# AllenNeuralDynamics/aind-smartspim-destripe

Measured on AMD Instinct MI355X. Metric: 2048x2048 uint16 slices/s destriped, higher is better.
Workload: dtype f32

## Files before the change

### aind_smartspim_destripe_amd/csrc/dsx_kernels.h

```cpp
#ifndef DSX_KERNELS_H
#define DSX_KERNELS_H

#include <type_traits>
#include <hip/hip_runtime.h>
#include <stdint.h>

#include "dsx_fft_core.h"

#ifndef DSX_NT
#define DSX_NT 1
#endif
#ifndef DSX_MEDIAN_BALLOT
#define DSX_MEDIAN_BALLOT 1
#endif
#ifndef DSX_FWD_STEADY
#define DSX_FWD_STEADY 1
#endif
#ifndef DSX_RF_XCD
#define DSX_RF_XCD 0
#endif
#ifndef DSX_INV_MINW
#define DSX_INV_MINW 1
#endif
#ifndef DSX_FWD_PRUNE
#define DSX_FWD_PRUNE 1
#endif
#ifndef DSX_SWZ
#define DSX_SWZ 1
#endif
#ifndef DSX_FWD_MINW
#define DSX_FWD_MINW 4
#endif


#ifdef DSX_DIAG
#define DSX_ABL(a, bits) (((a).ablate & (bits)) != 0)
#else
#define DSX_ABL(a, bits) false
#endif

namespace dsx {

constexpr int kMaxLevels = 16;
constexpr int kMaxPasses = 16;
constexpr int kWave = 64;

#define DSX_DEC_LO                                                                              \
  {0.03522629188570953f, -0.08544127388202666f, -0.13501102001025458f, 0.45987750211849154f,   \
   0.8068915093110925f,  0.33267055295008263f}
#define DSX_DEC_HI                                                                              \
  {-0.33267055295008263f, 0.8068915093110925f,  -0.45987750211849154f, -0.13501102001025458f,  \
   0.08544127388202666f,  0.03522629188570953f}
#define DSX_REC_LO                                                                              \
  {0.33267055295008263f,  0.8068915093110925f,   0.45987750211849154f, -0.13501102001025458f,  \
   -0.08544127388202666f, 0.03522629188570953f}
#define DSX_REC_HI                                                                              \
  {0.03522629188570953f, 0.08544127388202666f, -0.13501102001025458f, -0.45987750211849154f,   \
   0.8068915093110925f,  -0.33267055295008263f}

typedef unsigned dsx_u32x2 __attribute__((ext_vector_type(2)));
typedef float dsx_f2 __attribute__((ext_vector_type(2)));
typedef float dsx_f4 __attribute__((ext_vector_type(4)));
typedef unsigned dsx_u32x4 __attribute__((ext_vector_type(4)));

__device__ __forceinline__ __amdgpu_buffer_rsrc_t dsx_rsrc(const void* p) {
  return __builtin_amdgcn_make_buffer_rsrc((void*)p, 0, -1, 0x00020000);
}
constexpr int kBufNT = 2;

#if DSX_SCALAR_FMA
__device__ __forceinline__ dsx_f2 pk_fma(dsx_f2 a, dsx_f2 b, dsx_f2 c) { return dsx_f2{fmaf(a.x, b.x, c.x), fmaf(a.y, b.y, c.y)}; }
__device__ __forceinline__ dsx_f2 pk_fma(dsx_f2 a, float b, dsx_f2 c) { return dsx_f2{fmaf(a.x, b, c.x), fmaf(a.y, b, c.y)}; }
__device__ __forceinline__ dsx_f2 pk_fma(float a, dsx_f2 b, dsx_f2 c) { return dsx_f2{fmaf(a, b.x, c.x), fmaf(a, b.y, c.y)}; }
#else
__device__ __forceinline__ dsx_f2 pk_fma(dsx_f2 a, dsx_f2 b, dsx_f2 c) { return __builtin_elementwise_fma(a, b, c); }
__device__ __forceinline__ dsx_f2 pk_fma(dsx_f2 a, float b, dsx_f2 c) {
  const dsx_f2 bb = {b, b};
  return __builtin_elementwise_fma(a, bb, c);
}
__device__ __forceinline__ dsx_f2 pk_fma(float a, dsx_f2 b, dsx_f2 c) {
  const dsx_f2 aa = {a, a};
  return __builtin_elementwise_fma(aa, b, c);
}
#endif

struct PlaneStats {
  double sum_fg;
  double sum_all;
  unsigned long long cnt_fg;
  unsigned long long flags;
  unsigned pad_[56];
};
static_assert(sizeof(PlaneStats) == 256, "control block layout");

__device__ __forceinline__ int reflect_idx(int i, int n) {
  if (i >= 0 && i < n) return i;
  int p = 2 * n;
  i %= p;
  if (i < 0) i += p;
  return i < n ? i : p - 1 - i;
}

__device__ __forceinline__ float as_f32(unsigned u) { return __uint_as_float(u); }
__device__ __forceinline__ unsigned as_u32(float f) { return __float_as_uint(f); }

__device__ __forceinline__ double wave_sum_f64(double v) {
#pragma unroll
  for (int o = 32; o > 0; o >>= 1) v += __shfl_xor(v, o);
  return v;
}
__device__ __forceinline__ float wave_max_f32(float v) {
#pragma unroll
  for (int o = 32; o > 0; o >>= 1) v = fmaxf(v, __shfl_xor(v, o));
  return v;
}
__device__ __forceinline__ float wave_min_f32(float v) {
#pragma unroll
  for (int o = 32; o > 0; o >>= 1) v = fminf(v, __shfl_xor(v, o));
  return v;
}

__device__ __forceinline__ float min_no_nan(float a, float b) {
  float r;
  asm("v_min_f32 %0, %1, %2" : "=v"(r) : "v"(a), "v"(b));
  return r;
}
__device__ __forceinline__ float max_no_nan(float a, float b) {
  float r;
  asm("v_max_f32 %0, %1, %2" : "=v"(r) : "v"(a), "v"(b));
  return r;
}
__device__ __forceinline__ float wave_min_no_nan(float v) {
  v = min_no_nan(v, __builtin_bit_cast(float, __builtin_amdgcn_update_dpp(0, __builtin_bit_cast(int, v), 0xB1, 0xF, 0xF, true)));
  v = min_no_nan(v, __builtin_bit_cast(float, __builtin_amdgcn_update_dpp(0, __builtin_bit_cast(int, v), 0x4E, 0xF, 0xF, true)));
  v = min_no_nan(v, __builtin_bit_cast(float, __builtin_amdgcn_update_dpp(0, __builtin_bit_cast(int, v), 0x141, 0xF, 0xF, true)));
  v = min_no_nan(v, __builtin_bit_cast(float, __builtin_amdgcn_update_dpp(0, __builtin_bit_cast(int, v), 0x140, 0xF, 0xF, true)));
  const int b = __builtin_bit_cast(int, v);
  const float r0 = __builtin_bit_cast(float, __builtin_amdgcn_readlane(b, 0)), r1 = __builtin_bit_cast(float, __builtin_amdgcn_readlane(b, 16));
  const float r2 = __builtin_bit_cast(float, __builtin_amdgcn_readlane(b, 32)), r3 = __builtin_bit_cast(float, __builtin_amdgcn_readlane(b, 48));
  return fminf(fminf(r0, r1), fminf(r2, r3));
}

__device__ __forceinline__ unsigned swap_adjacent(unsigned v) {
  return (unsigned)__builtin_amdgcn_mov_dpp((int)v, 0xB1, 0xF, 0xF, true);
}

template <typename M>
__device__ __forceinline__ int slot_mask(M m, int e) {
  const unsigned w = (sizeof(M) == 8 && e >= 32) ? (unsigned)((unsigned long long)m >> 32) : (unsigned)m;
  return (int)(w << (31 - (e & 31))) >> 31;
}
template <typename M>
__device__ __forceinline__ M opaque_mask(M m) {
  if constexpr (sizeof(M) == 8) {
    unsigned lo = (unsigned)m, hi = (unsigned)((unsigned long long)m >> 32);
    asm volatile("" : "+v"(lo), "+v"(hi));
    return (M)(((unsigned long long)hi << 32) | lo);
  } else {
    unsigned lo = (unsigned)m;
    asm volatile("" : "+v"(lo));
    return (M)lo;
  }
}
__device__ __forceinline__ unsigned bit_select(int m, unsigned a, unsigned b) {
  unsigned r;
  asm("v_bfi_b32 %0, %1, %2, %3" : "=v"(r) : "v"(m), "v"(a), "v"(b));
  return r;
}
__device__ __forceinline__ int odd_lane_mask(int lane) {
  int m = -(lane & 1);
  asm("" : "+v"(m));
  return m;
}
__device__ __forceinline__ float bit_select(int m, float a, float b) {
  return as_f32(bit_select(m, as_u32(a), as_u32(b)));
}

__device__ __forceinline__ void wave_sync() {
  __builtin_amdgcn_fence(__ATOMIC_RELEASE, "wavefront");
  __builtin_amdgcn_wave_barrier();
  __builtin_amdgcn_fence(__ATOMIC_ACQUIRE, "wavefront");
}

#ifndef DSX_SCALAR_FMA
#define DSX_SCALAR_FMA 1
#endif
#ifndef DSX_FWD_PAIR
#define DSX_FWD_PAIR 1
#endif
#ifndef DSX_FWD_SPLIT
#define DSX_FWD_SPLIT 1
#endif
#ifndef DSX_DPP_X
#define DSX_DPP_X 1
#endif
__device__ __forceinline__ float lane_above(float v) {
  return __builtin_bit_cast(float, __builtin_amdgcn_update_dpp(0, __builtin_bit_cast(int, v), 0x130, 0xF, 0xF, true));
}

__global__ __launch_bounds__(256) void k_zero3(uint4* p0, int n0, uint4* p1, int n1, uint4* p2, int n2) {
  const uint4 z = make_uint4(0u, 0u, 0u, 0u);
  for (int i = blockIdx.x * 256 + threadIdx.x; i < n0 + n1 + n2; i += gridDim.x * 256) {
    if (i < n0) p0[i] = z;
    else if (i < n0 + n1) p1[i - n0] = z;
    else p2[i - n0 - n1] = z;
  }
}

struct Fwd1Args {
  const void* in;
  long long in_plane_stride;
  float* ws;
  long long ws_plane_stride;
  long long in_off;
  int H, W, ldin;
  long long aa_off, da_off;
  int h, w, ld, lda;
  unsigned* minmax;
  int lvl, L;
  PlaneStats* stats;
  float fg_cutoff;
  unsigned fg_cutoff_u16;
  int nstrips, nseg, rows_per_seg;
  long long aa2_off, da2_off;
  int h2, w2, ld2, lda2;
  int ablate;
  int shared;
};

constexpr int kMarchCols = 256;
constexpr int kMarchOut = (kMarchCols - 4) / 2;
constexpr int kFuseOut = (kMarchOut - 4) / 2;
constexpr int kRingRows = 8;
constexpr int kRingPitch = 128;
constexpr int kX2Pitch = 136;

template <int IN_KIND>
struct MarchStats {
  unsigned cnt = 0;
  unsigned isum_all = 0, isum_fg = 0;
  double fsum_all = 0.0, fsum_fg = 0.0;
  unsigned bad = 0;
  __device__ __forceinline__ void add(float f, float cutoff) {
    if (IN_KIND != 0) bad |= (f > -1.0f && f <= 3.402823466e38f) ? 0u : 1u;
    if (IN_KIND == 0) {
      const unsigned u = (unsigned)f;
      isum_all += u;
      if (f >= cutoff) { isum_fg += u; cnt++; }
    } else {
      fsum_all += (double)f;
      if (f >= cutoff) { fsum_fg += (double)f; cnt++; }
    }
  }
};

struct MarchRaw {
  float4 f;
};

struct MarchCol {
  int gc0;
  int base;
  bool vec;
  bool rev;
  bool dead;
  bool own;
  unsigned own_mask[2];
  int rc[4];
};

__device__ __forceinline__ MarchCol march_col(int gc0, int W, int ld, int w_out, bool lane_owns, bool ext) {
  MarchCol c;
  c.gc0 = gc0;
  c.own = lane_owns;
  c.dead = gc0 > 2 * w_out - 1;
  c.rev = false;
  c.base = gc0;
  const bool aligned = (ld & 3) == 0;
  c.vec = aligned && gc0 >= 0 && gc0 + 3 < W;
  if (ext && aligned && gc0 >= -4 && gc0 + 3 < W + 8) c.vec = true;
  if (!c.vec && !ext && aligned && (W & 3) == 0) {
    if (gc0 + 3 < 0 && -gc0 - 1 < W) { c.base = -gc0 - 4; c.rev = true; c.vec = true; }
    else if (gc0 >= W && 2 * W - 4 - gc0 >= 0) { c.base = 2 * W - 4 - gc0; c.rev = true; c.vec = true; }
  }
  if (c.dead) { c.base = 0; c.rev = false; }
  c.own_mask[0] = c.own_mask[1] = 0u;
#pragma unroll
  for (int e = 0; e < 4; ++e) {
    c.rc[e] = reflect_idx(gc0 + e, W);
    if (lane_owns && gc0 + e >= 0 && gc0 + e < W) c.own_mask[e >> 1] |= (e & 1) ? 0xFFFF0000u : 0x0000FFFFu;
  }
  return c;
}

template <int IN_KIND>
struct MarchSrc {
  static constexpr int ES = (IN_KIND == 0) ? 2 : 4;
  static constexpr int BIAS = (IN_KIND == 2) ? 4 : 0;
  const void* src;
  __amdgpu_buffer_rsrc_t rs;
  unsigned voff;
  __device__ __forceinline__ MarchSrc(const void* p, const MarchCol& c)
      : src(p), rs(dsx_rsrc((const char*)p - BIAS * ES)), voff((unsigned)(c.base + BIAS) * ES) {}
  __device__ __forceinline__ MarchRaw load(unsigned soff) const {
    MarchRaw r;
    if (IN_KIND == 0) {
      const dsx_u32x2 u = __builtin_amdgcn_raw_buffer_load_b64(rs, voff, soff, 0);
      r.f = make_float4(__uint_as_float(u.x), __uint_as_float(u.y), 0.f, 0.f);
    } else {
      const dsx_u32x4 u = __builtin_amdgcn_raw_buffer_load_b128(rs, voff, soff, 0);
      r.f = make_float4(__uint_as_float(u.x), __uint_as_float(u.y), __uint_as_float(u.z), __uint_as_float(u.w));
    }
    return r;
  }
};

// ... 903 lines not shown
template <int CPL, int M_, int S_, int R, int... REST>
__device__ __forceinline__ void fft_static_passes_swz(float2* buf, const float2* tw, int lane_in) {
  int lane = lane_in;
  asm volatile("" : "+v"(lane));
#if DSX_SWZ == 2
  fft_pass<R, CPL, (R - 1) / 2, (R - 1) / 2, dsx_idx_swz>(buf, tw, M_, S_, 1.0f / (float)S_, lane);
#else
  fft_pass_swz<R, CPL, M_, S_>(buf, tw, lane);
#endif
  if constexpr (sizeof...(REST) > 0) fft_static_passes_swz<CPL, M_, S_ * R, REST...>(buf, tw, lane_in);
}
template <int PLAN_>
struct StaticFft {
  static constexpr int M = 0;
  static constexpr bool kSwz = false;
};
template <>
struct StaticFft<1> {
  static constexpr int M = 1026;
  static constexpr bool kSwz = false;
  static constexpr int kRadix[3] = {19, 9, 6};
  template <int CPL>
  static __device__ __forceinline__ void run(float2* buf, const float2* tw, int lane) {
    fft_static_passes<CPL, 1026, 1, 19, 9, 6>(buf, tw, lane);
  }
#if DSX_FWD_PRUNE
  template <int CPL, int KO>
  static __device__ __forceinline__ void run_last_pruned(float2* buf, const float2* tw, int lane_in) {
    fft_static_passes<CPL, 1026, 1, 6, 9>(buf, tw, lane_in);
    int lane = lane_in;
    asm volatile("" : "+v"(lane));
    fft_pass<19, CPL, 9, KO>(buf, tw, 1026, 54, 1.0f / 54.0f, lane);
  }
  template <int CPL>
  static __device__ __forceinline__ void run_forward(float2* buf, const float2* tw, int lane, int kcut) {
    const int ko = (kcut + 53) / 54;
    if (ko <= 2) run_last_pruned<CPL, 2>(buf, tw, lane);
    else if (ko <= 4) run_last_pruned<CPL, 4>(buf, tw, lane);
    else run<CPL>(buf, tw, lane);
  }
#else
  template <int CPL>
  static __device__ __forceinline__ void run_forward(float2* buf, const float2* tw, int lane, int) { run<CPL>(buf, tw, lane); }
#endif
  template <int CPL, int JK>
  static __device__ __forceinline__ void run_first_pruned(float2* buf, const float2* tw, int lane_in) {
    int lane = lane_in;
    asm volatile("" : "+v"(lane));
    fft_pass<19, CPL, JK>(buf, tw, 1026, 1, 1.0f, lane);
    fft_static_passes<CPL, 1026, 19, 9, 6>(buf, tw, lane_in);
  }
  template <int CPL>
  static __device__ __forceinline__ void run_inverse(float2* buf, const float2* tw, int lane, int kcut) {
    const int jk = (kcut + 53) / 54;
    if (jk <= 2) run_first_pruned<CPL, 2>(buf, tw, lane);
    else if (jk <= 4) run_first_pruned<CPL, 4>(buf, tw, lane);
    else run<CPL>(buf, tw, lane);
  }
};
template <>
struct StaticFft<2> {
  static constexpr int M = 1071;
  static constexpr bool kSwz = false;
  static constexpr int kRadix[3] = {17, 9, 7};
  template <int CPL>
  static __device__ __forceinline__ void run(float2* buf, const float2* tw, int lane) {
    fft_static_passes<CPL, 1071, 1, 17, 9, 7>(buf, tw, lane);
  }
  template <int CPL>
  static __device__ __forceinline__ void run_forward(float2* buf, const float2* tw, int lane, int) { run<CPL>(buf, tw, lane); }
  template <int CPL>
  static __device__ __forceinline__ void run_inverse(float2* buf, const float2* tw, int lane, int) {
    run<CPL>(buf, tw, lane);
  }
};

#define DSX_STATIC_FFT(ID, LEN, R0, R1, R2, SWZ)                                                   \
  template <>                                                                                      \
  struct StaticFft<ID> {                                                                           \
    static constexpr int M = LEN;                                                                  \
    static constexpr bool kSwz = SWZ;                                                              \
    template <int CPL>                                                                             \
    static __device__ __forceinline__ void run(float2* buf, const float2* tw, int lane) {          \
      if constexpr (SWZ) fft_static_passes_swz<CPL, LEN, 1, R0, R1, R2>(buf, tw, lane);            \
      else fft_static_passes<CPL, LEN, 1, R0, R1, R2>(buf, tw, lane);                              \
    }                                                                                              \
    template <int CPL>                                                                             \
    static __device__ __forceinline__ void run_forward(float2* buf, const float2* tw, int lane, int) { \
      run<CPL>(buf, tw, lane);                                                                     \
    }                                                                                              \
    template <int CPL>                                                                             \
    static __device__ __forceinline__ void run_inverse(float2* buf, const float2* tw, int lane, int) { \
      run<CPL>(buf, tw, lane);                                                                     \
    }                                                                                              \
  };
DSX_STATIC_FFT(3, 2048, 16, 16, 8, DSX_SWZ != 0)
DSX_STATIC_FFT(4, 1815, 15, 11, 11, false)
DSX_STATIC_FFT(5, 1024, 16, 8, 8, DSX_SWZ != 0)
DSX_STATIC_FFT(6, 960, 15, 8, 8, false)
#undef DSX_STATIC_FFT

typedef short dsx_s16x2 __attribute__((ext_vector_type(2)));

__device__ __forceinline__ dsx_s16x2 as_s16x2(unsigned u) {
  union { unsigned u; dsx_s16x2 v; } c;
  c.u = u;
  return c.v;
}
__device__ __forceinline__ unsigned as_u32(dsx_s16x2 v) {
  union { unsigned u; dsx_s16x2 v; } c;
  c.v = v;
  return c.u;
}

template <int CPL>
struct RowSlots {
  static constexpr int GV = CPL / 4;
  static constexpr int E = 4 * GV + 4;
};
template <int E>
struct SlotMask { typedef unsigned long long type; };
template <> struct SlotMask<4> { typedef unsigned type; };
template <> struct SlotMask<8> { typedef unsigned type; };
template <> struct SlotMask<12> { typedef unsigned type; };
template <> struct SlotMask<20> { typedef unsigned type; };

template <int GV, typename F>
__device__ __forceinline__ void for_slots(int gf, int nt, F&& f) {
#pragma unroll
  for (int g = 0; g < GV; ++g) {
    if (g < gf) {
#pragma unroll
      for (int i = 0; i < 4; ++i) f(4 * g + i);
    }
  }
#pragma unroll
  for (int k = 0; k < 4; ++k) {
    if (k < nt) f(4 * GV + k);
  }
}

template <int GV, int E>
__device__ __forceinline__ unsigned count_below_pk16(const unsigned (&x)[E], unsigned t, int gf, int nt) {
  const dsx_s16x2 tv = as_s16x2(t);
  dsx_s16x2 acc = as_s16x2(0u);
  for_slots<GV>(gf, nt, [&](int e) {
    const dsx_s16x2 d = __builtin_elementwise_sub_sat(as_s16x2(x[e]), tv);
    acc -= (d >> 15);
  });
  return as_u32(acc);
}

template <int GV, int E>
__device__ __forceinline__ unsigned bisect_pk16(const unsigned (&x)[E], unsigned rank_a, unsigned rank_b,
                                                int gf, int nt) {
  unsigned ra = 0, rb = 0;
  for (int bit = 15; bit >= 0; --bit) {
    const unsigned ta = ra | (1u << bit), tb = rb | (1u << bit);
    unsigned c = count_below_pk16<GV, E>(x, (ta | (tb << 16)) ^ 0x80008000u, gf, nt);
    c = __reduce_add_sync(~0ull, c);
    if ((c & 0xFFFFu) <= rank_a) ra = ta;
    if ((c >> 16) <= rank_b) rb = tb;
  }
  return ra | (rb << 16);
}

template <int CPL>
constexpr int row_waves_per_simd() {
  return CPL <= 18 ? 4 : 1;
}
constexpr int kRowMaxWaves = 8;

__host__ __device__ __forceinline__ constexpr int rf_lds_row_b(int M) { return (M + 1) & ~1; }

template <int CPL, int GF_, int NT_, int HALO_, int PLAN_, bool TO_LDS>
__device__ __forceinline__ void rf_pair_body(const RowArgs& a, float2* s_tw, float2* buf, int tid, int nthreads, int lane,
                                             int pair, int plane) {
  const int M = (PLAN_ > 0) ? StaticFft<PLAN_>::M : a.M;
  constexpr bool SWZ = StaticFft<PLAN_>::kSwz;
  auto P = [](int i) { return SWZ ? dsx_idx_swz::at(i) : i; };
  const int N = a.w, K = (HALO_ == 0) ? 0 : a.K;
  const bool halo = (HALO_ >= 0) ? (HALO_ != 0) : (K > 0);
  const int npairs = (a.h + 1) >> 1;
  const bool live = pair < npairs;
  const int r0 = live ? 2 * pair : 0;
  const bool has_b = (r0 + 1) < a.h;
  const int cfg = a.cfg[plane];
  float* rowa = a.ws + plane * a.ws_plane_stride + a.da_off + (long long)r0 * a.ld;
  float* rowb = rowa + a.ld;

  constexpr int GV = RowSlots<CPL>::GV;
  constexpr int E = RowSlots<CPL>::E;
  typedef typename SlotMask<E>::type mask_t;
  const int gf = (GF_ >= 0) ? GF_ : (N >> 8);
  const int tail0 = gf << 8;
  const int nt = (NT_ >= 0) ? NT_ : ((N - tail0 + 63) >> 6);
  const int tn = tail0 + lane;

  const bool inactive = a.lvl >= a.lvl_active[cfg];
  auto zero_rows = [&]() {
    if (live) {
      for (int n = 4 * lane; n < N; n += 4 * kWave) {
        *(float4*)(rowa + n) = make_float4(0.f, 0.f, 0.f, 0.f);
        if (has_b) *(float4*)(rowb + n) = make_float4(0.f, 0.f, 0.f, 0.f);
      }
    }
  };
  if (!TO_LDS && inactive) {
    zero_rows();
    return;
  }
  const bool active = live && !inactive;
  const float thr = a.thr[(long long)plane * a.L + a.lvl];

  float4 ra4[GV > 0 ? GV : 1], rb4[GV > 0 ? GV : 1];
  float rta[4], rtb[4];
#pragma unroll
  for (int g = 0; g < GV; ++g) {
    ra4[g] = make_float4(0.f, 0.f, 0.f, 0.f);
    rb4[g] = make_float4(0.f, 0.f, 0.f, 0.f);
    if (active && g < gf) {
      ra4[g] = *(const float4*)(rowa + 256 * g + 4 * lane);
      if (has_b) rb4[g] = *(const float4*)(rowb + 256 * g + 4 * lane);
    }
  }
#pragma unroll
  for (int k = 0; k < 4; ++k) {
    rta[k] = 0.f;
    rtb[k] = 0.f;
    if (active && k < nt && tn + 64 * k < N) {
      rta[k] = rowa[tn + 64 * k];
      if (has_b) rtb[k] = rowb[tn + 64 * k];
    }
  }
  for (int i = tid; i < M; i += nthreads) s_tw[P(i)] = a.tw[i];
  __syncthreads();
  float* const lds_a = (float*)buf;
  float* const lds_b = (float*)buf + rf_lds_row_b(M);
  if (!active) {
    if (TO_LDS) {
      for (int n = 2 * lane; n < N; n += 2 * kWave) {
        *(float2*)(lds_a + n) = make_float2(0.f, 0.f);
        *(float2*)(lds_b + n) = make_float2(0.f, 0.f);
      }
    }
    return;
  }

  float va[E], vb[E];
  mask_t maska = 0, maskb = 0;
  auto take = [&](int e, float xa, float xb, bool valid) {
    const bool ma = valid && fabsf(xa) > thr, mb = valid && fabsf(xb) > thr;
    if (ma) maska |= ((mask_t)1 << e);
    if (mb) maskb |= ((mask_t)1 << e);
    va[e] = valid ? (ma ? 0.f : xa) : __builtin_huge_valf();
    vb[e] = valid ? (mb ? 0.f : xb) : __builtin_huge_valf();
  };
#pragma unroll
  for (int g = 0; g < GV; ++g) {
    if (g < gf) {
      take(4 * g + 0, ra4[g].x, rb4[g].x, true);
      take(4 * g + 1, ra4[g].y, rb4[g].y, true);
      take(4 * g + 2, ra4[g].z, rb4[g].z, true);
      take(4 * g + 3, ra4[g].w, rb4[g].w, true);
    }
  }
#pragma unroll
  for (int k = 0; k < 4; ++k) {
    if (k < nt) take(4 * GV + k, rta[k], rtb[k], tn + 64 * k < N);
  }
  if (!has_b) {
    for_slots<GV>(gf, nt, [&](int e) { if (vb[e] != __builtin_huge_valf()) vb[e] = 0.f; });
  }

  float meda = 0.f, medb = 0.f;
  const bool any_mask = __ballot((maska | maskb) != (mask_t)0) != 0ull;
  if (any_mask && !DSX_ABL(a, 1)) {
    const unsigned k1 = (unsigned)(N - 1) >> 1;
    const bool even = (N & 1) == 0;
    auto count2 = [&](float ta, float tb, bool le) -> unsigned {
#if DSX_MEDIAN_BALLOT
      unsigned ca = 0, cb = 0;
      for_slots<GV>(gf, nt, [&](int e) {
        ca += (unsigned)__popcll(__ballot(le ? (va[e] <= ta) : (va[e] < ta)));
        cb += (unsigned)__popcll(__ballot(le ? (vb[e] <= tb) : (vb[e] < tb)));
      });
      return ca | (cb << 16);
#else
      unsigned ca = 0, cb = 0;
      for_slots<GV>(gf, nt, [&](int e) {
        ca += (le ? (va[e] <= ta) : (va[e] < ta)) ? 1u : 0u;
        cb += (le ? (vb[e] <= tb) : (vb[e] < tb)) ? 1u : 0u;
      });
      return (unsigned)__builtin_amdgcn_readfirstlane((int)__reduce_add_sync(~0ull, ca | (cb << 16)));
#endif
    };
    float lo[2], hi[2];
    unsigned clo[2], chi[2];
    bool done[2];
    float flo[2], fhi[2];
    int last[2] = {0, 0};
    const float target = (float)k1 + 0.5f;
    const float thr_up = as_f32(as_u32(thr) + 1u);
    {
      const unsigned c0 = count2(0.f, 0.f, false), c0e = count2(0.f, 0.f, true);
#pragma unroll
      for (int r = 0; r < 2; ++r) {
        const unsigned lt = r ? (c0 >> 16) : (c0 & 0xFFFFu), le = r ? (c0e >> 16) : (c0e & 0xFFFFu);
        done[r] = false;
        if (k1 < lt) {
          lo[r] = -thr; clo[r] = 0u; hi[r] = 0.f; chi[r] = lt;
        } else if (k1 < le) {
          lo[r] = 0.f; clo[r] = lt; hi[r] = as_f32(1u); chi[r] = le; done[r] = true;
        } else {
          lo[r] = as_f32(1u); clo[r] = le; hi[r] = thr_up; chi[r] = (unsigned)N;
        }
        flo[r] = (float)clo[r] - target;
        fhi[r] = (float)chi[r] - target;
      }
    }
    bool adj[2] = {done[0], done[1]};
    for (int it = 0; it < 256; ++it) {
      const bool fin0 = adj[0] || chi[0] - clo[0] <= 1u, fin1 = adj[1] || chi[1] - clo[1] <= 1u;
      if (fin0 && fin1) break;
      float t[2];
#pragma unroll
      for (int r = 0; r < 2; ++r) {
        float tt = (lo[r] * fhi[r] - hi[r] * flo[r]) * __builtin_amdgcn_rcpf(fhi[r] - flo[r]);
        if ((it & 7) == 7 || !(tt > lo[r] && tt < hi[r])) {
          const unsigned kl = f32_key(lo[r]), kh = f32_key(hi[r]);
          if (kh - kl <= 1u) adj[r] = true;
          tt = key_f32(kl + ((kh - kl) >> 1));
        }
        t[r] = tt;
      }
      const unsigned c = count2(t[0], t[1], false);
#pragma unroll
      for (int r = 0; r < 2; ++r) {
        const unsigned cr = r ? (c >> 16) : (c & 0xFFFFu);
        const float f = (float)cr - target;
        if (cr <= k1) {
          lo[r] = t[r]; clo[r] = cr; flo[r] = f;
          if (last[r] == 1) fhi[r] *= 0.5f;
          last[r] = 1;
        } else {
          hi[r] = t[r]; chi[r] = cr; fhi[r] = f;
          if (last[r] == 2) flo[r] *= 0.5f;
          last[r] = 2;
        }
      }
    }
    float m_lo[2] = {__builtin_huge_valf(), __builtin_huge_valf()}, m_hi[2] = {__builtin_huge_valf(), __builtin_huge_valf()};
    for_slots<GV>(gf, nt, [&](int e) {
      m_lo[0] = min_no_nan(m_lo[0], va[e] >= lo[0] ? va[e] : __builtin_huge_valf());
      m_lo[1] = min_no_nan(m_lo[1], vb[e] >= lo[1] ? vb[e] : __builtin_huge_valf());
      if (even) {
        m_hi[0] = min_no_nan(m_hi[0], va[e] >= hi[0] ? va[e] : __builtin_huge_valf());
        m_hi[1] = min_no_nan(m_hi[1], vb[e] >= hi[1] ? vb[e] : __builtin_huge_valf());
      }
    });
    float sk[2], sk1[2];
#pragma unroll
    for (int r = 0; r < 2; ++r) {
      sk[r] = wave_min_no_nan(m_lo[r]);
      sk1[r] = sk[r];
      if (even) {
        const float nxt = wave_min_no_nan(m_hi[r]);
        sk1[r] = (k1 + 1u < chi[r]) ? sk[r] : nxt;
      }
    }
    meda = even ? 0.5f * (sk[0] + sk1[0]) : sk[0];
    medb = even ? 0.5f * (sk[1] + sk1[1]) : sk[1];
  }
  asm volatile("" : "+v"(meda), "+v"(medb));

  for_slots<GV>(gf, nt, [&](int e) {
    const int n = (e < 4 * GV) ? 256 * (e >> 2) + 4 * lane + (e & 3) : tn + 64 * (e - 4 * GV);
    if (e < 4 * GV || n < N) {
      const float xa = bit_select(slot_mask(maska, e), meda, va[e]);
      const float xb = bit_select(slot_mask(maskb, e), medb, vb[e]);
      const float2 z = make_float2(xa, xb);
      buf[P(K + n)] = z;
      if (halo) {
        if (n <= K) buf[P(K + N + n)] = z;
        if (n >= N - K) buf[P(n - (N - K))] = z;
      }
    }
  });
  if (halo) {
    for (int m = N + 2 * K + 1 + lane; m < M; m += kWave) buf[P(m)] = make_float2(0.f, 0.f);
  }
  wave_sync();

  if (!DSX_ABL(a, 2)) {
    if constexpr (PLAN_ > 0) StaticFft<PLAN_>::template run_forward<CPL>(buf, s_tw, lane, a.kcut[cfg]);
    else fft_run<CPL>(buf, s_tw, a, lane);
  }

  if (!DSX_ABL(a, 4)) {
    const float2* g1 = a.g[cfg];
    const float2* g2 = g1 + M;
    const int kcut = a.kcut[cfg];
    for (int k = lane; k <= kcut; k += kWave) {
      const int kr = (k == 0) ? 0 : M - k;
      const float2 u = buf[P(k)], ur = buf[P(kr)];
      const float ga = g1[k].x;
      const float2 gb = g2[k];
      const float2 v = make_float2(ga * u.x + gb.x * ur.x - gb.y * ur.y, ga * u.y + gb.x * ur.y + gb.y * ur.x);
      const float2 vr = make_float2(ga * ur.x + gb.x * u.x + gb.y * u.y, ga * ur.y + gb.x * u.y - gb.y * u.x);
      buf[P(k)] = make_float2(v.y, v.x);
      if (kr != k) buf[P(kr)] = make_float2(vr.y, vr.x);
    }
    for (int k = kcut + 1 + lane; k < M - kcut; k += kWave) buf[P(k)] = make_float2(0.f, 0.f);
    wave_sync();
  }

  if (!DSX_ABL(a, 2)) {
    if constexpr (PLAN_ > 0) StaticFft<PLAN_>::template run_inverse<CPL>(buf, s_tw, lane, a.kcut[cfg]);
    else fft_run<CPL>(buf, s_tw, a, lane);
  }

  maska = opaque_mask(maska);
  maskb = opaque_mask(maskb);
  if (TO_LDS) {
    float oa[E], ob[E];
    const int no_b = has_b ? 0 : -1;
    for_slots<GV>(gf, nt, [&](int e) {
      const int n = (e < 4 * GV) ? 256 * (e >> 2) + 4 * lane + (e & 3) : tn + 64 * (e - 4 * GV);
      oa[e] = 0.f;
      ob[e] = 0.f;
      if (e < 4 * GV || n < N) {
        const float2 y = buf[P(K + n)];
        oa[e] = bit_select(slot_mask(maska, e), 0.f, -y.y * a.inv_M);
        ob[e] = bit_select(slot_mask(maskb, e) | no_b, 0.f, -y.x * a.inv_M);
      }
    });
    wave_sync();
#pragma unroll
    for (int g = 0; g < GV; ++g) {
      if (g < gf) {
        const int nb0 = 256 * g + 4 * lane;
        *(float2*)(lds_a + nb0) = make_float2(oa[4 * g], oa[4 * g + 1]);
        *(float2*)(lds_a + nb0 + 2) = make_float2(oa[4 * g + 2], oa[4 * g + 3]);
        *(float2*)(lds_b + nb0) = make_float2(ob[4 * g], ob[4 * g + 1]);
        *(float2*)(lds_b + nb0 + 2) = make_float2(ob[4 * g + 2], ob[4 * g + 3]);
      }
    }
#pragma unroll
    for (int k = 0; k < 4; ++k) {
      const int n = tn + 64 * k;
      if (k < nt && n < N) {
        lds_a[n] = oa[4 * GV + k];
        lds_b[n] = ob[4 * GV + k];
      }
    }
    return;
  }
#pragma unroll
  for (int g = 0; g < GV; ++g) {
    if (g < gf) {
      const int nb0 = 256 * g + 4 * lane;
      float da_[4], db_[4];
#pragma unroll
      for (int i = 0; i < 4; ++i) {
        const int e = 4 * g + i;
        const float2 y = buf[P(K + nb0 + i)];
        da_[i] = bit_select(slot_mask(maska, e), 0.f, -y.y * a.inv_M);
        db_[i] = bit_select(slot_mask(maskb, e), 0.f, -y.x * a.inv_M);
      }
#if DSX_NT
      const dsx_f4 oa = {da_[0], da_[1], da_[2], da_[3]}, ob = {db_[0], db_[1], db_[2], db_[3]};
      __builtin_nontemporal_store(oa, (dsx_f4*)(rowa + nb0));
      if (has_b) __builtin_nontemporal_store(ob, (dsx_f4*)(rowb + nb0));
#else
      *(float4*)(rowa + nb0) = make_float4(da_[0], da_[1], da_[2], da_[3]);
      if (has_b) *(float4*)(rowb + nb0) = make_float4(db_[0], db_[1], db_[2], db_[3]);
#endif
    }
  }
#pragma unroll
  for (int k = 0; k < 4; ++k) {
    const int n = tn + 64 * k;
    if (k < nt && n < N) {
      const int e = 4 * GV + k;
      const float2 y = buf[P(K + n)];
      rowa[n] = bit_select(slot_mask(maska, e), 0.f, -y.y * a.inv_M);
      if (has_b) rowb[n] = bit_select(slot_mask(maskb, e), 0.f, -y.x * a.inv_M);
    }
  }
}

template <int CPL, int GF_ = -1, int NT_ = -1, int HALO_ = -1, int PLAN_ = 0>
__global__ __launch_bounds__(64 * kRowMaxWaves, row_waves_per_simd<CPL>()) void k_rowfilter(RowArgs a) {
  extern __shared__ __attribute__((aligned(16))) float2 dsx_smem[];
  const int tid = threadIdx.x, lane = tid & 63, wave = tid >> 6;
  const int M = (PLAN_ > 0) ? StaticFft<PLAN_>::M : a.M;
  rf_pair_body<CPL, GF_, NT_, HALO_, PLAN_, false>(a, dsx_smem, dsx_smem + (long long)M * (1 + wave), tid, blockDim.x, lane,
                                                   blockIdx.x * (blockDim.x >> 6) + wave, blockIdx.y);
}

constexpr int kRowMultiMax = 8;
struct RowMultiArgs {
  int nlev;
  int blk_end[kRowMultiMax];
  RowArgs lv[kRowMultiMax];
};

template <int CPL>
__global__ __launch_bounds__(64 * kRowMaxWaves, row_waves_per_simd<CPL>()) void k_rowfilter_multi(RowMultiArgs args) {
  extern __shared__ __attribute__((aligned(16))) float2 dsx_smem[];
  const int tid = threadIdx.x, lane = tid & 63, wave = tid >> 6;
  int ent = 0;
  while (ent + 1 < args.nlev && (int)blockIdx.x >= args.blk_end[ent]) ++ent;
  const RowArgs& a = args.lv[ent];
  const int bx = (int)blockIdx.x - (ent > 0 ? args.blk_end[ent - 1] : 0);
  rf_pair_body<CPL, -1, -1, -1, 0, false>(a, dsx_smem, dsx_smem + (long long)a.M * (1 + wave), tid, blockDim.x, lane,
                                          bx * (blockDim.x >> 6) + wave, blockIdx.y);
}

constexpr int kWideThreads = 512;
constexpr int kWideCpl = 36;
constexpr int kWideMaxLen = kWideThreads * kWideCpl;

__device__ __forceinline__ unsigned wide_block_sum(unsigned v, unsigned* s_red, int& turn) {
  v = __reduce_add_sync(~0ull, v);
  unsigned* slot = s_red + ((turn & 1) ? (kWideThreads / 64) : 0);
  if ((threadIdx.x & 63) == 0) slot[threadIdx.x >> 6] = v;
  __syncthreads();
  unsigned t = 0;
#pragma unroll
  for (int w = 0; w < kWideThreads / 64; ++w) t += slot[w];
  ++turn;
  return t;
}
__device__ __forceinline__ unsigned wide_block_min(unsigned v, unsigned* s_red, int& turn) {
  v = __reduce_min_sync(~0ull, v);
  unsigned* slot = s_red + ((turn & 1) ? (kWideThreads / 64) : 0);
  if ((threadIdx.x & 63) == 0) slot[threadIdx.x >> 6] = v;
  __syncthreads();
  unsigned t = ~0u;
#pragma unroll
  for (int w = 0; w < kWideThreads / 64; ++w) t = min(t, slot[w]);
  ++turn;
  return t;
}

template <int R, int CPL, int JK = (R - 1) / 2>
__device__ __forceinline__ void fft_pass_block(float2* buf, const float2* tw, int M, int s, float inv_s, int tid) {
  constexpr int MAXB = (CPL + R - 1) / R;
  const int nb = M / R;
  const bool unit_tw = (s * R == M);
  dsx_c32 v[MAXB][R];
#pragma unroll
  for (int i = 0; i < MAXB; ++i) {
    const int b = tid + kWideThreads * i;
    if (b < nb) dsx_bfly_load<R, JK>((const dsx_c32*)buf, b, nb, v[i]);
  }
  __syncthreads();
#pragma unroll
  for (int i = 0; i < MAXB; ++i) {
    const int b = tid + kWideThreads * i;
    if (b < nb) dsx_bfly_store<R, JK>((dsx_c32*)buf, (const dsx_c32*)tw, b, s, inv_s, v[i], unit_tw);
    __builtin_amdgcn_sched_barrier(0);
  }
  __syncthreads();
}
template <int CPL>
__device__ __forceinline__ void fft_pass_generic_block(float2* buf, const float2* tw, int M, int s, float inv_s, int R,
                                                       int tid) {
  float2 acc[CPL];
#pragma unroll
  for (int i = 0; i < CPL; ++i) {
    const int o = tid + kWideThreads * i;
    acc[i] = make_float2(0.f, 0.f);
    if (o < M) {
      const dsx_c32 r = dsx_generic_output((const dsx_c32*)buf, (const dsx_c32*)tw, o, M, s, inv_s, R);
      acc[i] = make_float2(r.x, r.y);
    }
  }
  __syncthreads();
#pragma unroll
  for (int i = 0; i < CPL; ++i) {
    const int o = tid + kWideThreads * i;
    if (o < M) buf[o] = acc[i];
  }
  __syncthreads();
}
template <int CPL>
__device__ __forceinline__ void fft_run_block(float2* buf, const float2* tw, const RowArgs& a, int tid_in) {
  int s = 1;
  for (int pi = 0; pi < a.npass; ++pi) {
    const int R = a.radix[pi];
    const float inv_s = 1.0f / (float)s;
    int tid = tid_in, M = a.M;
    asm volatile("" : "+v"(tid), "+s"(M));
    switch (R) {
      case 2: fft_pass_block<2, CPL>(buf, tw, M, s, inv_s, tid); break;
      case 3: fft_pass_block<3, CPL>(buf, tw, M, s, inv_s, tid); break;
      case 4: fft_pass_block<4, CPL>(buf, tw, M, s, inv_s, tid); break;
      case 5: fft_pass_block<5, CPL>(buf, tw, M, s, inv_s, tid); break;
      case 6: fft_pass_block<6, CPL>(buf, tw, M, s, inv_s, tid); break;
      case 8: fft_pass_block<8, CPL>(buf, tw, M, s, inv_s, tid); break;
      case 9: fft_pass_block<9, CPL>(buf, tw, M, s, inv_s, tid); break;
      case 10: fft_pass_block<10, CPL>(buf, tw, M, s, inv_s, tid); break;
      case 12: fft_pass_block<12, CPL>(buf, tw, M, s, inv_s, tid); break;
      case 15: fft_pass_block<15, CPL>(buf, tw, M, s, inv_s, tid); break;
      case 16: fft_pass_block<16, CPL>(buf, tw, M, s, inv_s, tid); break;
      case 20: fft_pass_block<20, CPL>(buf, tw, M, s, inv_s, tid); break;
      case 25: fft_pass_block<25, CPL>(buf, tw, M, s, inv_s, tid); break;
      case 7: fft_pass_block<7, CPL>(buf, tw, M, s, inv_s, tid); break;
      case 11: fft_pass_block<11, CPL>(buf, tw, M, s, inv_s, tid); break;
      case 13: fft_pass_block<13, CPL>(buf, tw, M, s, inv_s, tid); break;
      case 17: fft_pass_block<17, CPL>(buf, tw, M, s, inv_s, tid); break;
      case 19: fft_pass_block<19, CPL>(buf, tw, M, s, inv_s, tid); break;
      default: fft_pass_generic_block<CPL>(buf, tw, M, s, inv_s, R, tid); break;
    }
    s *= R;
  }
}

__global__ __launch_bounds__(kWideThreads) void k_rowfilter_wide(RowArgs a) {
  extern __shared__ __attribute__((aligned(16))) float2 dsx_smem[];
  __shared__ unsigned s_red[2 * (kWideThreads / 64)];
  constexpr int E = kWideCpl;
  float2* const buf = dsx_smem;
  const int tid = threadIdx.x, plane = blockIdx.y, pair = blockIdx.x;
  const int M = a.M, N = a.w, K = a.K;
  const bool halo = K > 0;
  const int r0 = 2 * pair;
  const bool has_b = (r0 + 1) < a.h;
  const int cfg = a.cfg[plane];
  float* rowa = a.ws + plane * a.ws_plane_stride + a.da_off + (long long)r0 * a.ld;
  float* rowb = rowa + a.ld;
  if (a.lvl >= a.lvl_active[cfg]) {
    for (int n = tid; n < N; n += kWideThreads) {
      rowa[n] = 0.f;
      if (has_b) rowb[n] = 0.f;
    }
    return;
  }
  const float thr = a.thr[(long long)plane * a.L + a.lvl];
  unsigned ka[E], kb[E];
  unsigned long long maska = 0ull, maskb = 0ull;
#pragma unroll
  for (int e = 0; e < E; ++e) {
    const int n = tid + kWideThreads * e;
    ka[e] = kb[e] = ~0u;
    if (n < N) {
      const float xa = rowa[n], xb = has_b ? rowb[n] : 0.f;
      const bool ma = fabsf(xa) > thr, mb = has_b && fabsf(xb) > thr;
      if (ma) maska |= 1ull << e;
      if (mb) maskb |= 1ull << e;
      ka[e] = f32_key(ma ? 0.f : xa);
      kb[e] = f32_key(mb ? 0.f : xb);
    }
  }
  int turn = 0;
  float meda = 0.f, medb = 0.f;
  const bool any_mask = wide_block_sum((maska | maskb) != 0ull ? 1u : 0u, s_red, turn) != 0u;
  if (any_mask) {
    const unsigned k1 = (unsigned)(N - 1) >> 1;
    auto count_below = [&](unsigned ta, unsigned tb) {
      unsigned c = 0;
#pragma unroll
      for (int e = 0; e < E; ++e) c += (ka[e] < ta ? 1u : 0u) + (kb[e] < tb ? 0x10000u : 0u);
      return wide_block_sum(c, s_red, turn);
    };
    unsigned pa = 0u, pb = 0u;
    for (int bit = 31; bit >= 0; --bit) {
      const unsigned ta = pa | (1u << bit), tb = pb | (1u << bit);
      const unsigned c = count_below(ta, tb);
      if ((c & 0xFFFFu) <= k1) pa = ta;
      if ((c >> 16) <= k1) pb = tb;
// ... 756 lines not shown
```

Before: 70850.

## Finish median selection with a 32-candidate window rank instead of full bracketing

Adds a windowed median path. The secant/bisection search now stops once the bracket holds at most 32 elements. Those candidates are compacted into shared memory with ballot/mbcnt, and each lane computes the rank of one candidate so the k-th and (k+1)-th values can be read directly. It also biases the secant step by an offset to cut stagnating iterations, replaces the initial zero counts with ballot popcounts, and skips the final min-reduction pass when it is not needed. The aim is fewer full passes over the row during median finding, at the cost of extra LDS traffic, wave syncs and more code complexity.

```diff
diff --git a/aind_smartspim_destripe_amd/csrc/dsx_kernels.h b/aind_smartspim_destripe_amd/csrc/dsx_kernels.h
--- a/aind_smartspim_destripe_amd/csrc/dsx_kernels.h
+++ b/aind_smartspim_destripe_amd/csrc/dsx_kernels.h
@@ -12,6 +12,9 @@
 #endif
 #ifndef DSX_MEDIAN_BALLOT
 #define DSX_MEDIAN_BALLOT 1
+#endif
+#ifndef DSX_MEDIAN_WINDOW
+#define DSX_MEDIAN_WINDOW 1
 #endif
 #ifndef DSX_FWD_STEADY
 #define DSX_FWD_STEADY 1
@@ -1521,8 +1524,31 @@
     int last[2] = {0, 0};
     const float target = (float)k1 + 0.5f;
     const float thr_up = as_f32(as_u32(thr) + 1u);
-    {
+#if DSX_MEDIAN_WINDOW
+    constexpr unsigned kWin = 32;
+    const unsigned win = M >= (int)kWin ? kWin : 1u;
+    const bool whole = (unsigned)N <= win;
+#else
+    constexpr bool whole = false;
+    constexpr unsigned win = 1;
+#endif
+    if (whole) {
+#pragma unroll
+      for (int r = 0; r < 2; ++r) {
+        lo[r] = -__builtin_huge_valf(); clo[r] = 0u; hi[r] = __builtin_huge_valf(); chi[r] = (unsigned)N; done[r] = false;
+        flo[r] = (float)clo[r] - target;
+        fhi[r] = (float)chi[r] - target;
+      }
+    } else {
+#if DSX_MEDIAN_WINDOW
+      unsigned c0 = 0, c0e = 0;
+      for_slots<GV>(gf, nt, [&](int e) {
+        c0 += (unsigned)__popcll(__ballot(va[e] < 0.f)) | ((unsigned)__popcll(__ballot(vb[e] < 0.f)) << 16);
+        c0e += (unsigned)__popcll(__ballot(va[e] <= 0.f)) | ((unsigned)__popcll(__ballot(vb[e] <= 0.f)) << 16);
+      });
+#else
       const unsigned c0 = count2(0.f, 0.f, false), c0e = count2(0.f, 0.f, true);
+#endif
 #pragma unroll
       for (int r = 0; r < 2; ++r) {
         const unsigned lt = r ? (c0 >> 16) : (c0 & 0xFFFFu), le = r ? (c0e >> 16) : (c0e & 0xFFFFu);
@@ -1540,12 +1566,17 @@
     }
     bool adj[2] = {done[0], done[1]};
     for (int it = 0; it < 256; ++it) {
-      const bool fin0 = adj[0] || chi[0] - clo[0] <= 1u, fin1 = adj[1] || chi[1] - clo[1] <= 1u;
+      const bool fin0 = adj[0] || chi[0] - clo[0] <= win, fin1 = adj[1] || chi[1] - clo[1] <= win;
       if (fin0 && fin1) break;
       float t[2];
 #pragma unroll
       for (int r = 0; r < 2; ++r) {
+#if DSX_MEDIAN_WINDOW
+        const float o = last[r] == 1 ? 4.f : (last[r] == 2 ? -4.f : 0.f);
+        float tt = (lo[r] * (fhi[r] - o) - hi[r] * (flo[r] - o)) * __builtin_amdgcn_rcpf(fhi[r] - flo[r]);
+#else
         float tt = (lo[r] * fhi[r] - hi[r] * flo[r]) * __builtin_amdgcn_rcpf(fhi[r] - flo[r]);
+#endif
         if ((it & 7) == 7 || !(tt > lo[r] && tt < hi[r])) {
           const unsigned kl = f32_key(lo[r]), kh = f32_key(hi[r]);
           if (kh - kl <= 1u) adj[r] = true;
@@ -1569,6 +1600,79 @@
         }
       }
     }
+#if DSX_MEDIAN_WINDOW
+    bool use_win[2], need_old = false;
+#pragma unroll
+    for (int r = 0; r < 2; ++r) {
+      use_win[r] = win == kWin && chi[r] - clo[r] <= kWin;
+      need_old = need_old || !use_win[r] || (even && k1 + 1u >= chi[r]);
+    }
+    float sel_k[2] = {0.f, 0.f}, sel_k1[2] = {0.f, 0.f};
+    if (use_win[0] || use_win[1]) {
+      float* const cand = (float*)buf;
+      unsigned base_a = 0, base_b = 0;
+      for_slots<GV>(gf, nt, [&](int e) {
+        const bool pa = va[e] >= lo[0] && va[e] < hi[0], pb = vb[e] >= lo[1] && vb[e] < hi[1];
+        const unsigned long long ba = __ballot(pa), bb = __ballot(pb);
+        const unsigned qa = __builtin_amdgcn_mbcnt_hi((unsigned)(ba >> 32), __builtin_amdgcn_mbcnt_lo((unsigned)ba, base_a));
+        const unsigned qb = __builtin_amdgcn_mbcnt_hi((unsigned)(bb >> 32), __builtin_amdgcn_mbcnt_lo((unsigned)bb, base_b));
+        if (pa && qa < kWin) cand[qa] = va[e];
+        if (pb && qb < kWin) cand[kWin + qb] = vb[e];
+        base_a += (unsigned)__popcll(ba);
+        base_b += (unsigned)__popcll(bb);
+      });
+      const unsigned h = (unsigned)lane >> 5, j = (unsigned)lane & (kWin - 1);
+      const unsigned ch_lo = h ? clo[1] : clo[0], nc = (h ? chi[1] : chi[0]) - ch_lo;
+      if (j >= nc) cand[lane] = __builtin_huge_valf();
+      wave_sync();
+      const float cj = cand[lane];
+      const float2* const c2 = (const float2*)(cand + kWin * h);
+      unsigned rank = 0;
+#pragma unroll
+      for (int q = 0; q < (int)kWin / 2; ++q) {
+        const float2 c = c2[q];
+        const float ci[2] = {c.x, c.y};
+#pragma unroll
+        for (int u = 0; u < 2; ++u) {
+          const unsigned i = 2 * q + u;
+          rank += (ci[u] < cj || (ci[u] == cj && i < j)) ? 1u : 0u;
+        }
+      }
+      const unsigned r1 = k1 - ch_lo;
+      const unsigned long long b1 = __ballot(rank == r1), b2 = __ballot(rank == r1 + 1u);
+      const int bits = __builtin_bit_cast(int, cj);
+      sel_k[0] = __builtin_bit_cast(float, __builtin_amdgcn_readlane(bits, __builtin_ctz((unsigned)b1 | 0x80000000u)));
+      sel_k[1] = __builtin_bit_cast(float, __builtin_amdgcn_readlane(bits, 32 + __builtin_ctz((unsigned)(b1 >> 32) | 0x80000000u)));
+      if (even) {
+        sel_k1[0] = __builtin_bit_cast(float, __builtin_amdgcn_readlane(bits, __builtin_ctz((unsigned)b2 | 0x80000000u)));
+        sel_k1[1] = __builtin_bit_cast(float, __builtin_amdgcn_readlane(bits, 32 + __builtin_ctz((unsigned)(b2 >> 32) | 0x80000000u)));
+      }
+      wave_sync();
+    }
+    float m_lo[2] = {__builtin_huge_valf(), __builtin_huge_valf()}, m_hi[2] = {__builtin_huge_valf(), __builtin_huge_valf()};
+    if (need_old) {
+      for_slots<GV>(gf, nt, [&](int e) {
+        m_lo[0] = min_no_nan(m_lo[0], va[e] >= lo[0] ? va[e] : __builtin_huge_valf());
+        m_lo[1] = min_no_nan(m_lo[1], vb[e] >= lo[1] ? vb[e] : __builtin_huge_valf());
+        if (even) {
+          m_hi[0] = min_no_nan(m_hi[0], va[e] >= hi[0] ? va[e] : __builtin_huge_valf());
+          m_hi[1] = min_no_nan(m_hi[1], vb[e] >= hi[1] ? vb[e] : __builtin_huge_valf());
+        }
+      });
+#pragma unroll
+      for (int r = 0; r < 2; ++r) {
+        m_lo[r] = wave_min_no_nan(m_lo[r]);
+        if (even) m_hi[r] = wave_min_no_nan(m_hi[r]);
+      }
+    }
+    float sk[2], sk1[2];
+#pragma unroll
+    for (int r = 0; r < 2; ++r) {
+      sk[r] = use_win[r] ? sel_k[r] : m_lo[r];
+      sk1[r] = sk[r];
+      if (even) sk1[r] = (k1 + 1u < chi[r]) ? (use_win[r] ? sel_k1[r] : sk[r]) : m_hi[r];
+    }
+#else
     float m_lo[2] = {__builtin_huge_valf(), __builtin_huge_valf()}, m_hi[2] = {__builtin_huge_valf(), __builtin_huge_valf()};
     for_slots<GV>(gf, nt, [&](int e) {
       m_lo[0] = min_no_nan(m_lo[0], va[e] >= lo[0] ? va[e] : __builtin_huge_valf());
@@ -1588,6 +1692,7 @@
         sk1[r] = (k1 + 1u < chi[r]) ? sk[r] : nxt;
       }
     }
+#endif
     meda = even ? 0.5f * (sk[0] + sk1[0]) : sk[0];
     medb = even ? 0.5f * (sk[1] + sk1[1]) : sk[1];
   }
```

Measured after the change: 73220, median of 6. 3.3% higher.
